# DarylFernandes99/custom-yolo-implmentation

Measured on AMD Instinct MI355X. Metric: images/sec (640x640 bf16), higher is better.
Workload: dtype bf16; 1 GPU; preset s (width 32..512, depth 1) 640x640 train step (fwd+DFL/QFL loss+bwd+grad sync+AdamW), COCO-80 synthetic, 32 img/GPU; global_batch=32, parallelism=dp1, hip_graph=True, optimizer_in_graph=True, deterministic_mode=False

## Files before the change

custom-yolo-implmentation_amd/csrc/conv_mfma.hip:

```cpp
#include <cstdio>
#include <cstdlib>
#include "common.h"
#include "conv_geom.h"
#include "conv_dev.h"

int halo_conv_eligible(const ConvGeom& g);
int rows_conv_eligible(const ConvGeom& g);
int rows_conv_launch(const ConvGeom& g, int variant, const void* src, const void* wm, const float* bias, void* dst, int accumulate,
                     int dtype, hipStream_t st);
int halo_conv_launch(const ConvGeom& g, int variant, const void* src, const void* wm, const float* bias, void* dst,
                     int accumulate, int dtype, hipStream_t st);

ConvTune& conv_tune() {
    static ConvTune t = [] {
        ConvTune v{0, -1, -1, -1, -1, 0, 0, 0};
        if (const char* e = getenv("YOLO_CONV_TUNE"))
            sscanf(e, "%d,%d,%d,%d,%d,%d,%d,%d", &v.bn, &v.tap_inner, &v.halo, &v.dma, &v.ring, &v.bm, &v.nst, &v.bk);
        return v;
    }();
    return t;
}

int ring_conv_eligible(const ConvGeom& g, int dtype, const void* src, const void* wm, const void* dst);
int ring_conv_plan(const ConvGeom* gs, int n);
int ring_conv_launch(const ConvGeom* gs, int n, const long* wm_off, long wm_elems, const void* src, const void* wm,
                     const float* bias, void* dst, int accumulate, int dtype, hipStream_t st);

namespace {

template <typename T, int WGM, int WGN, int WM, int WN, bool ACC, int MODE>
__global__ __launch_bounds__(256) __attribute__((amdgpu_waves_per_eu(4, 8))) void k_conv_mfma(GeomDev g, const T* __restrict__ src, const T* __restrict__ wm,
                                                   const float* __restrict__ bias, T* __restrict__ dst, int ntile_n) {
    static_assert(WGM * WGN == 4 && WGM * WM * 16 == BM, "tile shape");
    constexpr int BN = WGN * WN * 16;
    using ops = mfma_ops<T>;
    using frag = typename ops::frag;
    __shared__ __attribute__((aligned(16))) T lds_a[2][BM][LDSROW];
    __shared__ __attribute__((aligned(16))) T lds_b[2][BN][LDSROW];

    const int tid = threadIdx.x, lane = tid & 63, wave = tid >> 6;
    const int nwg = gridDim.x;
    const int tile = xcd_remap(blockIdx.x, nwg);
    const int tile_m = tile / ntile_n, tile_n = tile - tile_m * ntile_n;
    const int m0 = tile_m * BM;
    const int cd0 = tile_n * BN;
    const int total_pix = g.N * g.Hg * g.Wg;

    const int kseg = tid & 3;
    const int lrow = tid >> 2;
    const int sk = (kseg ^ ((-(lrow >> 2)) & 3)) * 8;
    int rowoff[2], hs0[2], ws0[2];
#pragma unroll
    for (int i = 0; i < 2; ++i) {
        const int q = m0 + lrow + i * 64;
        const bool rv = q < total_pix;
        const unsigned qq = rv ? q : 0;
        const unsigned t2 = qq / (unsigned)g.Wg, b = qq - t2 * g.Wg;
        const unsigned n = t2 / (unsigned)g.Hg, a = t2 - n * g.Hg;
        hs0[i] = rv ? (int)a * g.sstride : -(1 << 20);
        ws0[i] = (int)b * g.sstride;
        rowoff[i] = (((int)n * g.Hs + (int)a * g.sstride) * g.Ws + (int)b * g.sstride) * g.lds;
    }
    constexpr int WR = (BN + 63) / 64;
    bool wvalid[WR];
#pragma unroll
    for (int i = 0; i < WR; ++i) {
        const int r = lrow + i * 64;
        wvalid[i] = (r < BN) && (cd0 + r < g.Cd);
    }

    uint4 ra[2], rb[WR];

    unsigned vmask[2] = {0u, 0u};
    int voffa[2], voffb[WR];
    int tap = 0, cbase = 0, wcol = 0;
    __amdgpu_buffer_rsrc_t rsa, rsb;
    int ltap = 0, ch = kseg * 8;
    const T* wrow[WR];

    if constexpr (MODE >= 2) {
        for (int t = 0; t < g.ntaps; ++t) {
            const int dh = (int)((g.dh_pack >> (2 * t)) & 3u) - 1, dw = (int)((g.dw_pack >> (2 * t)) & 3u) - 1;
#pragma unroll
            for (int i = 0; i < 2; ++i) {
                const bool ok = (unsigned)(hs0[i] + dh) < (unsigned)g.Hs && (unsigned)(ws0[i] + dw) < (unsigned)g.Ws;
                vmask[i] |= (ok ? 1u : 0u) << t;
            }
        }
        const int shift = (g.Ws + 1) * g.lds;
        rsa = __builtin_amdgcn_make_buffer_rsrc(const_cast<T*>(src) - shift, 0, (g.N * g.Hs * g.Ws * g.lds + shift) * 2,
                                                0x00020000);
        rsb = __builtin_amdgcn_make_buffer_rsrc(const_cast<T*>(wm), 0, g.Cd * g.Kpad * 2, 0x00020000);
        const int kload = MODE == 3 ? (kseg ^ ((-(lrow >> 2)) & 3)) : kseg;
#pragma unroll
        for (int i = 0; i < 2; ++i) voffa[i] = (rowoff[i] + kload * 8) * 2;
#pragma unroll
        for (int i = 0; i < WR; ++i)
            voffb[i] = wvalid[i] ? ((cd0 + lrow + i * 64) * g.Kpad + kload * 8) * 2 : (int)0x80000000;
    } else {
#pragma unroll
        for (int i = 0; i < WR; ++i) wrow[i] = wm + (long)(cd0 + (wvalid[i] ? lrow + i * 64 : 0)) * g.Kpad + kseg * 8;
        while (ch >= g.Cs) { ch -= g.Cs; ++ltap; }
    }

    auto gload = [&](int kt) {
        if constexpr (MODE >= 2) {
            const int soff = ((int)((g.dh_pack >> (2 * tap)) & 3u) * g.Ws + (int)((g.dw_pack >> (2 * tap)) & 3u)) * g.lds + cbase;
#pragma unroll
            for (int i = 0; i < 2; ++i) {
                const int vo = ((vmask[i] >> tap) & 1u) ? voffa[i] : (int)0x80000000;
                const u32x4 v = __builtin_amdgcn_raw_buffer_load_b128(rsa, vo, soff * 2, 0);
                ra[i] = make_uint4(v.x, v.y, v.z, v.w);
            }
#pragma unroll
            for (int i = 0; i < WR; ++i) {
                const u32x4 v = __builtin_amdgcn_raw_buffer_load_b128(rsb, voffb[i], wcol * 2, 0);
                rb[i] = make_uint4(v.x, v.y, v.z, v.w);
            }
            if (g.tap_inner) {
                ++tap;
                wcol += g.Cs;
                if (tap == g.ntaps) { tap = 0; cbase += BK; wcol += BK - g.ntaps * g.Cs; }
            } else {
                cbase += BK;
                wcol += BK;
                if (cbase == g.Cs) { cbase = 0; ++tap; }
            }
        } else {
            const bool tv = ltap < g.ntaps;
            const int dh = (int)((g.dh_pack >> (2 * ltap)) & 3u) - 1, dw = (int)((g.dw_pack >> (2 * ltap)) & 3u) - 1;
            const int tapoff = (dh * g.Ws + dw) * g.lds + ch;
#pragma unroll
            for (int i = 0; i < 2; ++i) {
                const bool ok = tv && (unsigned)(hs0[i] + dh) < (unsigned)g.Hs && (unsigned)(ws0[i] + dw) < (unsigned)g.Ws;
                const uint4 v = *reinterpret_cast<const uint4*>(src + (ok ? rowoff[i] + tapoff : 0));
                ra[i] = ok ? v : make_uint4(0, 0, 0, 0);
            }
#pragma unroll
            for (int i = 0; i < WR; ++i) {
                const uint4 v = *reinterpret_cast<const uint4*>(wrow[i] + kt * BK);
                rb[i] = wvalid[i] ? v : make_uint4(0, 0, 0, 0);
            }
            ch += BK;
            if (MODE == 1) { while (ch >= g.Cs) { ch -= g.Cs; ++ltap; } }
            else if (ch >= g.Cs) { ch -= g.Cs; ++ltap; }
        }
    };
    auto gload_dma = [&](int buf) {
        const int soff = ((int)((g.dh_pack >> (2 * tap)) & 3u) * g.Ws + (int)((g.dw_pack >> (2 * tap)) & 3u)) * g.lds + cbase;
#pragma unroll
        for (int i = 0; i < 2; ++i) {
            const int vo = ((vmask[i] >> tap) & 1u) ? voffa[i] : (int)0x80000000;
            lds_dma16(rsa, &lds_a[buf][wave * 16 + i * 64][0], vo, soff * 2);
        }
#pragma unroll
        for (int i = 0; i < WR; ++i)
            if (BN >= (i + 1) * 64 || wave * 16 + i * 64 < BN)
                lds_dma16(rsb, &lds_b[buf][wave * 16 + i * 64][0], voffb[i], wcol * 2);
        if (g.tap_inner) {
            ++tap;
            wcol += g.Cs;
            if (tap == g.ntaps) { tap = 0; cbase += BK; wcol += BK - g.ntaps * g.Cs; }
        } else {
            cbase += BK;
            wcol += BK;
            if (cbase == g.Cs) { cbase = 0; ++tap; }
        }
    };
    auto lstore = [&](int buf) {
#pragma unroll
        for (int i = 0; i < 2; ++i)
            *reinterpret_cast<uint4*>(&lds_a[buf][lrow + i * 64][sk]) = ra[i];
#pragma unroll
        for (int i = 0; i < WR; ++i)
            if (BN >= (i + 1) * 64 || lrow + i * 64 < BN) *reinterpret_cast<uint4*>(&lds_b[buf][lrow + i * 64][sk]) = rb[i];
    };

    const int wgm = wave / WGN, wgn = wave - wgm * WGN;
    const int prow = wgm * WM * 16, crow = wgn * WN * 16;
    const int fr = lane & 15;
    const int fk = ((lane >> 4) ^ ((-(fr >> 2)) & 3)) * 8;
    f32x4 acc[WM][WN];
#pragma unroll
    for (int i = 0; i < WM; ++i)
#pragma unroll
        for (int j = 0; j < WN; ++j) acc[i][j] = (f32x4){0.f, 0.f, 0.f, 0.f};

    if constexpr (MODE == 3) {
        gload_dma(0);
        asm volatile("s_waitcnt vmcnt(0)" ::: "memory");
        __syncthreads();
        for (int kt = 0; kt < g.KT; ++kt) {
            const int buf = kt & 1;
            if (kt + 1 < g.KT) gload_dma(buf ^ 1);
            frag fa[WN], fb[WM];
#pragma unroll
            for (int j = 0; j < WN; ++j) fa[j] = *reinterpret_cast<const frag*>(&lds_b[buf][crow + j * 16 + fr][fk]);
#pragma unroll
            for (int i = 0; i < WM; ++i) fb[i] = *reinterpret_cast<const frag*>(&lds_a[buf][prow + i * 16 + fr][fk]);
#pragma unroll
            for (int i = 0; i < WM; ++i)
#pragma unroll
                for (int j = 0; j < WN; ++j) acc[i][j] = ops::mma(fa[j], fb[i], acc[i][j]);
            asm volatile("s_waitcnt vmcnt(0)" ::: "memory");
            __syncthreads();
        }
    } else {
        gload(0);
        lstore(0);
        __syncthreads();
        for (int kt = 0; kt < g.KT; ++kt) {
            const int buf = kt & 1;
            if (kt + 1 < g.KT) gload(kt + 1);
            frag fa[WN], fb[WM];
#pragma unroll
            for (int j = 0; j < WN; ++j) fa[j] = *reinterpret_cast<const frag*>(&lds_b[buf][crow + j * 16 + fr][fk]);
#pragma unroll
            for (int i = 0; i < WM; ++i) fb[i] = *reinterpret_cast<const frag*>(&lds_a[buf][prow + i * 16 + fr][fk]);
#pragma unroll
            for (int i = 0; i < WM; ++i)
#pragma unroll
                for (int j = 0; j < WN; ++j) acc[i][j] = ops::mma(fa[j], fb[i], acc[i][j]);
            if (kt + 1 < g.KT) lstore(buf ^ 1);
            __syncthreads();
        }
    }

    const int cq = (lane >> 4) * 4;
    float bv[WN][4];
#pragma unroll
    for (int j = 0; j < WN; ++j) {
        const int c = cd0 + crow + j * 16 + cq;
#pragma unroll
        for (int r = 0; r < 4; ++r) bv[j][r] = (bias != nullptr && c < g.Cd) ? bias[c + r] : 0.f;
    }
    {
        int q = m0 + prow + fr;
        const unsigned qq = q < total_pix ? q : 0;
        const unsigned t2 = qq / (unsigned)g.Wg;
        int b = (int)(qq - t2 * g.Wg);
        int n = (int)(t2 / (unsigned)g.Hg);
        int a = (int)t2 - n * g.Hg;
#pragma unroll
        for (int i = 0; i < WM; ++i) {
            const bool live = q < total_pix;
            const long pix = live ? ((long)n * g.Hd + a * g.ostep + g.ooff_h) * (long)g.Wd + b * g.ostep + g.ooff_w : 0;
            store_pixel_blocks<T, WN, ACC>(g, acc[i], bv, dst, pix, live, cd0 + crow, cq, lane);
            q += 16;
            b += 16;
            while (b >= g.Wg) {
                b -= g.Wg;
                if (++a == g.Hg) { a = 0; ++n; }
            }
        }
    }

    float* const stats = g.stats;
    if (stats != nullptr) {
        float* sacc = reinterpret_cast<float*>(&lds_a[0][0][0]);
        for (int t = tid; t < 2 * BN; t += 256) sacc[t] = 0.f;
        __syncthreads();
#pragma unroll
        for (int j = 0; j < WN; ++j) {
            float s[4] = {0.f, 0.f, 0.f, 0.f}, q2[4] = {0.f, 0.f, 0.f, 0.f};
#pragma unroll
            for (int i = 0; i < WM; ++i)
#pragma unroll
                for (int r = 0; r < 4; ++r) {
                    const float v = to_f<T>(from_f<T>(acc[i][j][r]));
                    s[r] += v;
                    q2[r] += v * v;
                }
#pragma unroll
            for (int r = 0; r < 4; ++r) {
                s[r] = row16_sum(s[r]);
                q2[r] = row16_sum(q2[r]);
            }
            if (fr == 0) {
                const int cl = crow + j * 16 + cq;
#pragma unroll
                for (int r = 0; r < 4; ++r) {
                    atomicAdd(&sacc[cl + r], s[r]);
                    atomicAdd(&sacc[BN + cl + r], q2[r]);
                }
            }
        }
        __syncthreads();
        float* o = stats + (long)(blockIdx.x & 7) * 2 * g.Cd;
        for (int t = tid; t < BN; t += 256)
            if (cd0 + t < g.Cd) {
                atomicAdd(o + cd0 + t, sacc[t]);
                atomicAdd(o + g.Cd + cd0 + t, sacc[BN + t]);
            }
    }
}

constexpr int WG_BP = 32;
constexpr int WG_LDSROW = 40;

template <typename T>
__global__ __launch_bounds__(256) void k_wgrad_mfma(const T* __restrict__ x, int ldx, const T* __restrict__ dy, int ldy,
                                                    float* __restrict__ dwp, int Kpad, int N, int H, int W, int Cin,
                                                    int OH, int OW, int Cout, int k, int stride, int ci_tiles,
                                                    long slab_pix) {
    using ops = mfma_ops<T>;
    using frag = typename ops::frag;
    __shared__ __attribute__((aligned(16))) T lds_y[64][WG_LDSROW];
    __shared__ __attribute__((aligned(16))) T lds_x[64][WG_LDSROW];

    const int tid = threadIdx.x, lane = tid & 63, wave = tid >> 6;
    const int co0 = blockIdx.x * 64;
    const int tapi = blockIdx.y / ci_tiles;
    const int ci0 = (blockIdx.y - tapi * ci_tiles) * 64;
    const int kh = tapi / k, kw = tapi - kh * k, pad = k / 2;
    const long P = (long)N * OH * OW;
    const long q0 = (long)blockIdx.z * slab_pix;
    long q1 = q0 + slab_pix;
    if (q1 > P) q1 = P;
    const int steps = (int)((q1 - q0 + WG_BP - 1) / WG_BP);

    const int pix = tid & 31, seg = tid >> 5;
    const bool yv = co0 + seg * 8 < Cout, xv = ci0 + seg * 8 < Cin;

    uint4 ry, rx;
    auto gload = [&](int s) {
        long q = q0 + (long)s * WG_BP + pix;
        ry = make_uint4(0, 0, 0, 0);
        rx = make_uint4(0, 0, 0, 0);
        if (q < q1) {
            int ow = (int)(q % OW);
            long t2 = q / OW;
            int oh = (int)(t2 % OH);
            long n = t2 / OH;
            if (yv) ry = *reinterpret_cast<const uint4*>(dy + q * ldy + co0 + seg * 8);
            int ih = oh * stride + kh - pad, iw = ow * stride + kw - pad;
            if (xv && ih >= 0 && ih < H && iw >= 0 && iw < W)
                rx = *reinterpret_cast<const uint4*>(x + ((n * H + ih) * (long)W + iw) * ldx + ci0 + seg * 8);
        }
    };
    auto lstore = [&]() {
        const T* py = reinterpret_cast<const T*>(&ry);
        const T* px = reinterpret_cast<const T*>(&rx);
#pragma unroll
        for (int j = 0; j < 8; ++j) {
            lds_y[seg * 8 + j][pix] = py[j];
            lds_x[seg * 8 + j][pix] = px[j];
        }
    };

    const int wc = wave >> 1, wi = wave & 1;
    const int fr = lane & 15, fk = (lane >> 4) * 8;
    f32x4 acc[2][2];
#pragma unroll
    for (int i = 0; i < 2; ++i)
#pragma unroll
        for (int j = 0; j < 2; ++j) acc[i][j] = (f32x4){0.f, 0.f, 0.f, 0.f};

    if (steps > 0) gload(0);
    for (int s = 0; s < steps; ++s) {
        __syncthreads();
        lstore();
        __syncthreads();
        if (s + 1 < steps) gload(s + 1);
        frag fa[2], fb[2];
#pragma unroll
        for (int i = 0; i < 2; ++i) fa[i] = *reinterpret_cast<const frag*>(&lds_y[wc * 32 + i * 16 + fr][fk]);
#pragma unroll
        for (int j = 0; j < 2; ++j) fb[j] = *reinterpret_cast<const frag*>(&lds_x[wi * 32 + j * 16 + fr][fk]);
#pragma unroll
        for (int i = 0; i < 2; ++i)
#pragma unroll
            for (int j = 0; j < 2; ++j) acc[i][j] = ops::mma(fa[i], fb[j], acc[i][j]);
    }

#pragma unroll
    for (int i = 0; i < 2; ++i)
#pragma unroll
        for (int j = 0; j < 2; ++j) {
            int ci = ci0 + wi * 32 + j * 16 + fr;
            if (ci >= Cin) continue;
#pragma unroll
            for (int r = 0; r < 4; ++r) {
                int co = co0 + wc * 32 + i * 16 + (lane >> 4) * 4 + r;
                if (co < Cout) atomicAdd(dwp + (long)co * Kpad + tapi * Cin + ci, acc[i][j][r]);
            }
        }
}

template <typename T, int WGM, int WGN, int WM, int WN>
void launch_tile(const GeomDev& d, const void* src, const void* wm, const float* bias, void* dst, int accumulate,
                 hipStream_t st) {
    constexpr int BN = WGN * WN * 16;
    long pix = (long)d.N * d.Hg * d.Wg;
    int tm = (int)((pix + BM - 1) / BM), tn = (d.Cd + BN - 1) / BN;
    dim3 grid(tm * tn);
    int mode = d.Cs < BK ? 1 : (d.Cs % BK == 0 ? 2 : 0);
    if (mode == 2 && d.dma) mode = 3;
#define CONV_LAUNCH(ACC_, SM_)                                                                                        \
    hipLaunchKernelGGL((k_conv_mfma<T, WGM, WGN, WM, WN, ACC_, SM_>), grid, dim3(256), 0, st, d, (const T*)src,       \
                       (const T*)wm, bias, (T*)dst, tn)
    if (accumulate) { if (mode == 1) CONV_LAUNCH(true, 1); else if (mode == 2) CONV_LAUNCH(true, 2); else if (mode == 3) CONV_LAUNCH(true, 3); else CONV_LAUNCH(true, 0); }
    else { if (mode == 1) CONV_LAUNCH(false, 1); else if (mode == 2) CONV_LAUNCH(false, 2); else if (mode == 3) CONV_LAUNCH(false, 3); else CONV_LAUNCH(false, 0); }
#undef CONV_LAUNCH
}

int conv_tile_bn(const GeomDev& d_in) {
    const long tm = ((long)d_in.N * d_in.Hg * d_in.Wg + BM - 1) / BM;
    auto blocks = [&](int bn) { return tm * ((d_in.Cd + bn - 1) / bn); };
    int bn = d_in.Cd > 64 ? 128 : (d_in.Cd > 32 ? 64 : 32);
    const long src_bytes = (long)d_in.N * d_in.Hs * d_in.Ws * d_in.lds * 2;
    if (bn == 128 && d_in.ntaps == 1 && src_bytes <= (128L << 20)) bn = 64;
    while (bn > 32 && blocks(bn) < 256) bn >>= 1;
    const ConvTune& tu = conv_tune();
    if (tu.bn == 32 || tu.bn == 64 || tu.bn == 128) bn = tu.bn;
    return bn;
}

template <typename T>
void launch_conv_t(const GeomDev& d_in, const void* src, const void* wm, const float* bias, void* dst, int accumulate,
                   hipStream_t st) {
    const int bn = conv_tile_bn(d_in);
    GeomDev d = d_in;
    const ConvTune& tu = conv_tune();
    if (tu.tap_inner >= 0) d.tap_inner = tu.tap_inner;
    if (tu.dma >= 0) d.dma = tu.dma;
    if (bn == 128) launch_tile<T, 2, 2, 4, 4>(d, src, wm, bias, dst, accumulate, st);
    else if (bn == 64) launch_tile<T, 2, 2, 4, 2>(d, src, wm, bias, dst, accumulate, st);
    else launch_tile<T, 4, 1, 2, 2>(d, src, wm, bias, dst, accumulate, st);
}

bool al16(const void* p) { return (reinterpret_cast<uintptr_t>(p) & 15) == 0; }

}

extern "C" int yolo_conv_tune_set(int bn, int tap_inner, int halo, int dma, int ring, int bm, int nst, int bk) {
    ConvTune& t = conv_tune();
    t.bn = bn; t.tap_inner = tap_inner; t.halo = halo; t.dma = dma; t.ring = ring; t.bm = bm; t.nst = nst; t.bk = bk;
    return YOLO_OK;
}

static int& wide_state() {
    static int v = [] { const char* e = getenv("YOLO_CONV_WIDE"); const int m = e ? atoi(e) : 2; return m < 0 ? 0 : m > 2 ? 2 : m; }();
    return v;
}
int conv_wide_flag() { return wide_state(); }
extern "C" int yolo_conv_wide_set(int on) { wide_state() = on < 0 ? 0 : on > 2 ? 2 : on; return YOLO_OK; }

int mfma_conv_eligible(const ConvGeom& g, int dtype, const void* src, const void* wm, const void* dst) {
    if (dtype != YOLO_BF16 && dtype != YOLO_F16) return 0;
    if (g.Cs % 8 || g.lds % 8 || g.Cd % 8 || g.ldd % 4) return 0;
    if ((long)g.N * g.Hs * g.Ws * g.lds + (long)(g.Ws + 1) * g.lds >= (1L << 30)) return 0;
    if ((long)g.N * g.Hg * g.Wg + 256 >= (1L << 31) || (long)g.Cd * g.Kpad >= (1L << 30)) return 0;
    if (!al16(src) || !al16(wm) || (reinterpret_cast<uintptr_t>(dst) & 7)) return 0;
    for (int t = 0; t < g.ntaps; ++t)
        if (g.dh[t] < -1 || g.dh[t] > 1 || g.dw[t] < -1 || g.dw[t] > 1) return 0;
    return 1;
}

static int halo_variant(const ConvGeom& g) {
    const int v = conv_tune().halo;
    if (!halo_conv_eligible(g)) return 0;
    if (v >= 0 && v <= 4) return v;
    if ((long)g.Hg * g.Wg >= 80 * 80) return g.Cd >= 128 ? 2 : 3;
    if (g.Hg >= 40 && g.Wg >= 40 && g.Cd == 128) return 1;
    return 0;
}

static int rows_variant(const ConvGeom& g) {
    const int v = conv_tune().halo;
    const int el = rows_conv_eligible(g);
    if (!el) return 0;
    if ((v >= 0 && v < 5) || v == 9) return 0;
    if (el == 3) return (v == 16 || ((v < 0 || v == 5) && g.Cs % 32 == 0)) ? 7 : 0;
    if (v == 14) return 6;
    if (el != 1) return (v < 0 || v == 5) && g.Cd == 64 && g.Cs >= 64 ? 6 : 0;
    if (v == 6) return 1;
    if (v == 7) return g.Cd > 64 ? 2 : 1;
    if (v == 8) return 3;
    if (v == 12) return 4;
    if (g.Wg == 40) return 4;
    const long wgs = (long)g.N * ((g.Hg + 3) / 4) * ((g.Cd + 63) / 64);
    return wgs >= 512 ? 4 : 3;
}

int mfma_conv_plan(const ConvGeom& g, int dtype) {
    static const long long dummy[2] = {0, 0};
    if (const int rv = rows_variant(g)) return 4000 + rv;
    if (const int hv = halo_variant(g)) return 2000 + hv;
    if (ring_conv_eligible(g, dtype, dummy, dummy, dummy)) return ring_conv_plan(&g, 1);
    return 1000 + conv_tile_bn(to_dev(g));
}

int mfma_conv_launch(const ConvGeom& g, const void* src, const void* wm, const float* bias, void* dst, int accumulate,
                     int dtype, hipStream_t st) {
    if ((long)g.N * g.Hg * g.Wg == 0) return YOLO_OK;
    if (const int rv = rows_variant(g)) return rows_conv_launch(g, rv, src, wm, bias, dst, accumulate, dtype, st);
    if (const int hv = halo_variant(g)) return halo_conv_launch(g, hv, src, wm, bias, dst, accumulate, dtype, st);
    if (ring_conv_eligible(g, dtype, src, wm, dst)) {
        const long off0 = 0;
        return ring_conv_launch(&g, 1, &off0, (long)g.Cd * g.Kpad, src, wm, bias, dst, accumulate, dtype, st);
    }
    GeomDev d = to_dev(g);
    if (dtype == YOLO_BF16) launch_conv_t<bf16_t>(d, src, wm, bias, dst, accumulate, st);
    else launch_conv_t<f16_t>(d, src, wm, bias, dst, accumulate, st);
    return YOLO_LAUNCH_CHECK();
}

int mfma_wgrad_eligible(int Cin, int Cout, int ldx, int ldy, int dtype, const void* x, const void* dy) {
    if (dtype != YOLO_BF16 && dtype != YOLO_F16) return 0;
    if (Cin % 8 || Cout % 8 || ldx % 8 || ldy % 8) return 0;
    return al16(x) && al16(dy);
}

int mfma_wgrad_launch(const void* x, int ldx, const void* dy, int ldy, float* dwp, int Kpad, int N, int H, int W,
                      int Cin, int OH, int OW, int Cout, int k, int stride, int dtype, hipStream_t st) {
    long P = (long)N * OH * OW;
    if (P == 0) return YOLO_OK;
    int cot = (Cout + 63) / 64, cit = (Cin + 63) / 64, nt = k * k;
    long tiles = (long)cot * cit * nt;
    long max_slabs = 4096 / tiles;
    if (max_slabs < 1) max_slabs = 1;
    long slab = (P + max_slabs - 1) / max_slabs;
    if (slab < 1024) slab = 1024;
    slab = (slab + WG_BP - 1) / WG_BP * WG_BP;
    int nslab = (int)((P + slab - 1) / slab);
    dim3 grid(cot, cit * nt, nslab);
    if (dtype == YOLO_BF16)
        hipLaunchKernelGGL((k_wgrad_mfma<bf16_t>), grid, dim3(256), 0, st, (const bf16_t*)x, ldx, (const bf16_t*)dy, ldy,
                           dwp, Kpad, N, H, W, Cin, OH, OW, Cout, k, stride, cit, slab);
    else
        hipLaunchKernelGGL((k_wgrad_mfma<f16_t>), grid, dim3(256), 0, st, (const f16_t*)x, ldx, (const f16_t*)dy, ldy,
                           dwp, Kpad, N, H, W, Cin, OH, OW, Cout, k, stride, cit, slab);
    return YOLO_LAUNCH_CHECK();
}
```

Measured before the change: 3062 images/s.

## Add weight-resident persistent 1x1 conv kernel for large low-channel layers

Adds a new 1x1 convolution kernel that loads the full weight panel for a tile of output channels into LDS once. Each persistent workgroup then streams many 128-pixel activation blocks through a 4-slot LDS ring using buffer-load-to-LDS DMA. It is enabled by default for large-pixel-count 1x1 convs with small input channels, aiming to cut repeated weight loads and per-tile launch overhead. The trade-offs are higher LDS use, which may lower occupancy, and a fixed grid sized from the CU count, which may leave some CUs with uneven work.

Result: no change. 3066 images/s, median of 5 (+0.1%).

```diff
diff --git a/custom-yolo-implmentation_amd/csrc/conv_mfma.hip b/custom-yolo-implmentation_amd/csrc/conv_mfma.hip
--- a/custom-yolo-implmentation_amd/csrc/conv_mfma.hip
+++ b/custom-yolo-implmentation_amd/csrc/conv_mfma.hip
@@ -10,6 +10,9 @@
                      int dtype, hipStream_t st);
 int halo_conv_launch(const ConvGeom& g, int variant, const void* src, const void* wm, const float* bias, void* dst,
                      int accumulate, int dtype, hipStream_t st);
+int wres_conv_eligible(const ConvGeom& g, int bn);
+int wres_conv_launch(const ConvGeom& g, int bn, const void* src, const void* wm, const float* bias, void* dst, int accumulate,
+                     int dtype, hipStream_t st);
 
 ConvTune& conv_tune() {
     static ConvTune t = [] {
@@ -457,8 +460,13 @@
     return 1;
 }
 
+static int family_tune() {
+    const int v = conv_tune().halo;
+    return v >= 20 ? -1 : v;
+}
+
 static int halo_variant(const ConvGeom& g) {
-    const int v = conv_tune().halo;
+    const int v = family_tune();
     if (!halo_conv_eligible(g)) return 0;
     if (v >= 0 && v <= 4) return v;
     if ((long)g.Hg * g.Wg >= 80 * 80) return g.Cd >= 128 ? 2 : 3;
@@ -467,7 +475,7 @@
 }
 
 static int rows_variant(const ConvGeom& g) {
-    const int v = conv_tune().halo;
+    const int v = family_tune();
     const int el = rows_conv_eligible(g);
     if (!el) return 0;
     if ((v >= 0 && v < 5) || v == 9) return 0;
@@ -483,8 +491,25 @@
     return wgs >= 512 ? 4 : 3;
 }
 
+static int wres_default_on() {
+    static const int v = [] { const char* e = getenv("YOLO_CONV_WRES"); return e ? atoi(e) != 0 : 1; }();
+    return v;
+}
+static int wres_variant(const ConvGeom& g) {
+    const ConvTune& tu = conv_tune();
+    const int v = tu.halo;
+    if (v >= 0 && v <= 20) return 0;
+    if (v >= 22 && v <= 24) return wres_conv_eligible(g, 32 << (v - 22));
+    if (v == 21) return wres_conv_eligible(g, 0);
+    if (!wres_default_on() || tu.bn != 0 || tu.ring == 1) return 0;
+    if ((long)g.N * g.Hg * g.Wg < 100000) return 0;
+    if (!(g.Cs <= 96 || (g.Cd >= 256 && g.Cs <= 192))) return 0;
+    return wres_conv_eligible(g, 0);
+}
+
 int mfma_conv_plan(const ConvGeom& g, int dtype) {
     static const long long dummy[2] = {0, 0};
+    if (const int wv = wres_variant(g)) return 6000 + wv;
     if (const int rv = rows_variant(g)) return 4000 + rv;
     if (const int hv = halo_variant(g)) return 2000 + hv;
     if (ring_conv_eligible(g, dtype, dummy, dummy, dummy)) return ring_conv_plan(&g, 1);
@@ -494,6 +519,7 @@
 int mfma_conv_launch(const ConvGeom& g, const void* src, const void* wm, const float* bias, void* dst, int accumulate,
                      int dtype, hipStream_t st) {
     if ((long)g.N * g.Hg * g.Wg == 0) return YOLO_OK;
+    if (const int wv = wres_variant(g)) return wres_conv_launch(g, wv, src, wm, bias, dst, accumulate, dtype, st);
     if (const int rv = rows_variant(g)) return rows_conv_launch(g, rv, src, wm, bias, dst, accumulate, dtype, st);
     if (const int hv = halo_variant(g)) return halo_conv_launch(g, hv, src, wm, bias, dst, accumulate, dtype, st);
     if (ring_conv_eligible(g, dtype, src, wm, dst)) {
diff --git a/custom-yolo-implmentation_amd/csrc/conv_wres.hip b/custom-yolo-implmentation_amd/csrc/conv_wres.hip
--- /dev/null
+++ b/custom-yolo-implmentation_amd/csrc/conv_wres.hip
@@ -0,0 +1,241 @@
+#include "conv_dev.h"
+
+namespace {
+
+__device__ __forceinline__ void wres_dma(__amdgpu_buffer_rsrc_t rs, unsigned lds_addr, int voff, int soff) {
+    asm volatile("s_mov_b32 m0, %0\n\ts_nop 0\n\tbuffer_load_dwordx4 %1, %2, %3 offen lds"
+                 :: "s"(lds_addr), "v"(voff), "s"(rs), "s"(soff) : "memory");
+}
+template <int N> __device__ __forceinline__ void wres_wait() { asm volatile("s_waitcnt vmcnt(%0) lgkmcnt(0)" :: "n"(N) : "memory"); }
+
+constexpr int WRES_BMP = 128;
+constexpr int WRES_NSLOT = 4;
+constexpr int WRES_SLOT = WRES_BMP * 64;
+
+template <typename T, int WGM, int WGN, int WM, int WN, bool ACC>
+__global__ __launch_bounds__(256) void k_conv_wres(GeomDev g, const T* __restrict__ src, const T* __restrict__ wm,
+                                                   const float* __restrict__ bias, T* __restrict__ dst, int ntile_n, int nblk, int G) {
+    static_assert(WGM * WGN == 4 && WGM * WM * 16 == WRES_BMP, "tile shape");
+    constexpr int BN = WGN * WN * 16, NSLOT = WRES_NSLOT, SLOT = WRES_SLOT;
+    constexpr int AP = WRES_BMP / 16 / 4;
+    constexpr int RB = BN / 16;
+    constexpr int OOB = (int)0x80000000;
+    using ops = mfma_ops<T>;
+    using frag = typename ops::frag;
+    extern __shared__ __attribute__((aligned(1024))) char wres_smem[];
+    const unsigned lds0 = __builtin_amdgcn_readfirstlane((unsigned)(size_t)(__attribute__((address_space(3))) char*)wres_smem);
+
+    const int tid = threadIdx.x, lane = tid & 63, wave = __builtin_amdgcn_readfirstlane(tid >> 6);
+    const int tile = xcd_remap(blockIdx.x, gridDim.x);
+    const int gi = tile / ntile_n, tile_n = tile - gi * ntile_n;
+    const int cd0 = tile_n * BN;
+    const int b0 = (int)((long)gi * nblk / G), b1 = (int)((long)(gi + 1) * nblk / G);
+    const int P = g.N * g.Hg * g.Wg;
+    const int nchunk = g.KT;
+    const int nsteps = (b1 - b0) * nchunk;
+
+    {
+        const __amdgpu_buffer_rsrc_t rsb = __builtin_amdgcn_make_buffer_rsrc(const_cast<T*>(wm), 0, g.Cd * g.Kpad * 2, 0x00020000);
+        const int npiece = RB * nchunk;
+        for (int p = wave; p < npiece; p += 4) {
+            const int c = p / RB, row = (p - c * RB) * 16 + (lane >> 2);
+            const int kseg = (lane & 3) ^ ((-(row >> 2)) & 3);
+            const bool ok = cd0 + row < g.Cd && c * BK + kseg * 8 < g.Cs;
+            wres_dma(rsb, lds0 + NSLOT * SLOT + p * 1024, ok ? ((cd0 + row) * g.Kpad + c * BK + kseg * 8) * 2 : OOB, 0);
+        }
+    }
+
+    const int a_bytes = P * g.lds * 2;
+    int avoff[AP], apx[AP];
+#pragma unroll
+    for (int i = 0; i < AP; ++i) {
+        const int px = (wave * AP + i) * 16 + (lane >> 2), ck = (lane & 3) ^ ((-(px >> 2)) & 3);
+        apx[i] = px;
+        avoff[i] = ck * 8 < g.Cs ? (px * g.lds + ck * 8) * 2 : OOB;
+    }
+    int istep = 0, iblk = b0, ichunk = 0, islot = 0;
+    auto issue = [&]() {
+        const __amdgpu_buffer_rsrc_t rsa = __builtin_amdgcn_make_buffer_rsrc(const_cast<T*>(src), 0, istep < nsteps ? a_bytes : 0, 0x00020000);
+        const int q0 = iblk * WRES_BMP;
+        const int soff = __builtin_amdgcn_readfirstlane((q0 * g.lds + ichunk * BK) * 2);
+        const unsigned base = __builtin_amdgcn_readfirstlane(lds0 + islot * SLOT + wave * (AP * 1024));
+#pragma unroll
+        for (int i = 0; i < AP; ++i) wres_dma(rsa, base + i * 1024, q0 + apx[i] < P ? avoff[i] : OOB, soff);
+        ++istep;
+        if (++ichunk == nchunk) { ichunk = 0; ++iblk; }
+        if (++islot == NSLOT) islot = 0;
+    };
+
+    const int wgm = wave / WGN, wgn = wave - wgm * WGN;
+    const int prow = wgm * WM * 16, crow = wgn * WN * 16;
+    const int fr = lane & 15, fg = lane >> 4, cq = fg * 4;
+    const int fk = (fg ^ ((-(fr >> 2)) & 3)) * 16;
+    const int aoff = (prow + fr) * 64 + fk;
+    const int boff = NSLOT * SLOT + (crow + fr) * 64 + fk;
+    f32x4 acc[WM][WN];
+    float ssum[WN][4], ssq[WN][4];
+#pragma unroll
+    for (int j = 0; j < WN; ++j)
+#pragma unroll
+        for (int r = 0; r < 4; ++r) ssum[j][r] = ssq[j][r] = 0.f;
+#pragma unroll
+    for (int i = 0; i < WM; ++i)
+#pragma unroll
+        for (int j = 0; j < WN; ++j) acc[i][j] = (f32x4){0.f, 0.f, 0.f, 0.f};
+    float bv[WN][4];
+#pragma unroll
+    for (int j = 0; j < WN; ++j) {
+        const int c = cd0 + crow + j * 16 + cq;
+#pragma unroll
+        for (int r = 0; r < 4; ++r) bv[j][r] = (bias != nullptr && c < g.Cd) ? bias[c + r] : 0.f;
+    }
+#pragma unroll
+    for (int j = 0; j < WN; ++j)
+#pragma unroll
+        for (int r = 0; r < 4; ++r) asm volatile("" : "+v"(bv[j][r]));
+    float* const stats = g.stats;
+
+#pragma unroll
+    for (int s = 0; s < NSLOT - 1; ++s) issue();
+    int rslot = 0, chunk = 0, q0 = b0 * WRES_BMP;
+    for (int step = 0; step < nsteps; ++step) {
+        wres_wait<(NSLOT - 2) * AP>();
+        __builtin_amdgcn_s_barrier();
+        issue();
+        const char* ap = wres_smem + rslot * SLOT + aoff;
+        const char* bp = wres_smem + chunk * (BN * 64) + boff;
+        frag fa[WN], fb[WM];
+#pragma unroll
+        for (int j = 0; j < WN; ++j) fa[j] = *reinterpret_cast<const frag*>(bp + j * 1024);
+#pragma unroll
+        for (int i = 0; i < WM; ++i) fb[i] = *reinterpret_cast<const frag*>(ap + i * 1024);
+#pragma unroll
+        for (int i = 0; i < WM; ++i)
+#pragma unroll
+            for (int j = 0; j < WN; ++j) acc[i][j] = ops::mma(fa[j], fb[i], acc[i][j]);
+        if (++rslot == NSLOT) rslot = 0;
+        if (++chunk == nchunk) {
+            chunk = 0;
+#pragma unroll
+            for (int i = 0; i < WM; ++i) {
+                const int q = q0 + prow + i * 16 + fr;
+                const bool live = q < P;
+                store_pixel_blocks<T, WN, ACC>(g, acc[i], bv, dst, live ? (long)q : 0, live, cd0 + crow, cq, lane);
+            }
+            if (stats != nullptr) {
+#pragma unroll
+                for (int j = 0; j < WN; ++j)
+#pragma unroll
+                    for (int i = 0; i < WM; ++i)
+#pragma unroll
+                        for (int r = 0; r < 4; ++r) {
+                            const float v = to_f<T>(from_f<T>(acc[i][j][r]));
+                            ssum[j][r] += v;
+                            ssq[j][r] += v * v;
+                        }
+            }
+#pragma unroll
+            for (int i = 0; i < WM; ++i)
+#pragma unroll
+                for (int j = 0; j < WN; ++j) acc[i][j] = (f32x4){0.f, 0.f, 0.f, 0.f};
+            q0 += WRES_BMP;
+        }
+    }
+    wres_wait<0>();
+    __syncthreads();
+
+    if (stats != nullptr) {
+        float* sacc = reinterpret_cast<float*>(wres_smem);
+        for (int t = tid; t < 2 * BN; t += 256) sacc[t] = 0.f;
+        __syncthreads();
+#pragma unroll
+        for (int j = 0; j < WN; ++j) {
+#pragma unroll
+            for (int r = 0; r < 4; ++r) {
+                ssum[j][r] = row16_sum(ssum[j][r]);
+                ssq[j][r] = row16_sum(ssq[j][r]);
+            }
+            if (fr == 0) {
+                const int cl = crow + j * 16 + cq;
+#pragma unroll
+                for (int r = 0; r < 4; ++r) {
+                    atomicAdd(&sacc[cl + r], ssum[j][r]);
+                    atomicAdd(&sacc[BN + cl + r], ssq[j][r]);
+                }
+            }
+        }
+        __syncthreads();
+        float* o = stats + (long)(blockIdx.x & 7) * 2 * g.Cd;
+        for (int t = tid; t < BN; t += 256)
+            if (cd0 + t < g.Cd) {
+                atomicAdd(o + cd0 + t, sacc[t]);
+                atomicAdd(o + g.Cd + cd0 + t, sacc[BN + t]);
+            }
+    }
+}
+
+int wres_cus() {
+    static int cus[64] = {0};
+    int dev = 0;
+    if (hipGetDevice(&dev) != hipSuccess) return 256;
+    int& c = cus[dev & 63];
+    if (c == 0) {
+        int v = 0;
+        c = (hipDeviceGetAttribute(&v, hipDeviceAttributeMultiprocessorCount, dev) == hipSuccess && v > 0) ? v : 256;
+    }
+    return c;
+}
+
+template <typename T, int WGM, int WGN, int WM, int WN>
+int launch_wres(const GeomDev& d, const void* src, const void* wm, const float* bias, void* dst, int accumulate, hipStream_t st) {
+    constexpr int BN = WGN * WN * 16;
+    const size_t lds = (size_t)WRES_NSLOT * WRES_SLOT + (size_t)d.KT * BN * 64;
+    const long P = (long)d.N * d.Hg * d.Wg;
+    const int nblk = (int)((P + WRES_BMP - 1) / WRES_BMP), tn = (d.Cd + BN - 1) / BN;
+    constexpr int wreg = BN == 128 ? 2 : BN == 64 ? 3 : 4;
+    int wpc = (int)((160u << 10) / lds);
+    wpc = wpc < 1 ? 1 : wpc > wreg ? wreg : wpc;
+    int G = wres_cus() * wpc / tn;
+    if (G > nblk / 2) G = nblk / 2;
+    if (G < 1) G = 1;
+    const dim3 grid((unsigned)(G * tn));
+    if (accumulate) {
+        static unsigned long long done = 0;
+        if (int e = yolo_allow_dyn_lds(reinterpret_cast<const void*>(k_conv_wres<T, WGM, WGN, WM, WN, true>), lds, done)) return e;
+        hipLaunchKernelGGL((k_conv_wres<T, WGM, WGN, WM, WN, true>), grid, dim3(256), lds, st, d, (const T*)src, (const T*)wm, bias, (T*)dst, tn, nblk, G);
+    } else {
+        static unsigned long long done = 0;
+        if (int e = yolo_allow_dyn_lds(reinterpret_cast<const void*>(k_conv_wres<T, WGM, WGN, WM, WN, false>), lds, done)) return e;
+        hipLaunchKernelGGL((k_conv_wres<T, WGM, WGN, WM, WN, false>), grid, dim3(256), lds, st, d, (const T*)src, (const T*)wm, bias, (T*)dst, tn, nblk, G);
+    }
+    return YOLO_LAUNCH_CHECK();
+}
+
+}
+
+int wres_conv_eligible(const ConvGeom& g, int bn) {
+    if (!(g.ntaps == 1 && g.dh[0] == 0 && g.dw[0] == 0 && g.sstride == 1 && g.ostep == 1 && g.ooff_h == 0 && g.ooff_w == 0 &&
+          (g.Cs % 32 == 0 || g.Cs == 16) && g.Cd % 8 == 0 && g.lds % 8 == 0 && g.Hg == g.Hs && g.Wg == g.Ws && g.Hd == g.Hg && g.Wd == g.Wg))
+        return 0;
+    if (g.Kpad != round_up32(g.Cs)) return 0;
+    if ((long)g.N * g.Hg * g.Wg < 2 * WRES_BMP) return 0;
+    if (((long)g.N * g.Hg * g.Wg + WRES_NSLOT * WRES_BMP) * g.lds >= (1L << 30)) return 0;
+    auto panel = [&](int b) { return (long)b * g.Kpad * 2; };
+    if (bn != 32 && bn != 64 && bn != 128) {
+        bn = g.Cd > 64 ? 128 : (g.Cd > 32 ? 64 : 32);
+        while (bn > 32 && panel(bn) + WRES_NSLOT * WRES_SLOT > (80L << 10)) bn >>= 1;
+    }
+    return panel(bn) <= (96L << 10) ? bn : 0;
+}
+
+int wres_conv_launch(const ConvGeom& g, int bn, const void* src, const void* wm, const float* bias, void* dst, int accumulate,
+                     int dtype, hipStream_t st) {
+    const GeomDev d = to_dev(g);
+#define WRES_T(T_)                                                                                                   \
+    if (bn == 128) return launch_wres<T_, 2, 2, 4, 4>(d, src, wm, bias, dst, accumulate, st);    \
+    if (bn == 64) return launch_wres<T_, 2, 2, 4, 2>(d, src, wm, bias, dst, accumulate, st);            \
+    return launch_wres<T_, 4, 1, 2, 2>(d, src, wm, bias, dst, accumulate, st);
+    if (dtype == YOLO_BF16) { WRES_T(bf16_t) }
+    WRES_T(f16_t)
+#undef WRES_T
+}
```
